# brownvc/matryodshka

Measured on AMD Instinct MI355X. Metric: novel-view frames/sec, 640x320 ODS->32-sphere MSI infer+render, higher is better.
Workload: dtype f32

## Files before the change

include/msi_hip.h:

```cpp
#ifndef MSI_HIP_H
#define MSI_HIP_H

#include <stddef.h>
#include <stdint.h>

#ifdef __cplusplus
extern "C" {
#endif

#define MSI_OK 0
#define MSI_E_BADARG (-1)
#define MSI_E_LAUNCH (-2)
#define MSI_E_UNSUPPORTED (-3)
#define MSI_E_WORKSPACE (-4)
#define MSI_E_RANGE (-5)

typedef void *msi_stream_t;

const char *msi_version(void);
#define MSI_ABI_VERSION 9
int32_t msi_abi_version(void);
const char *msi_last_error_string(void);
uint32_t msi_crc32c_host(const void *data_host, size_t n, uint32_t crc);

// ... 150 lines not shown
  uint64_t param_offset;
  uint64_t param_floats;
  uint64_t raw_offset;
  uint64_t affine_offset;
  uint64_t ln_scale_offset;
} msi_layer_info;

int msi_net_layer_info(const msi_net_desc *desc, int32_t layer, msi_layer_info *out);
size_t msi_net_param_floats(const msi_net_desc *desc);
size_t msi_net_packed_floats(const msi_net_desc *desc);
int msi_net_pack_weights_host(const msi_net_desc *desc, const float *params_host,
                              float *packed_host);
size_t msi_net_workspace_bytes(const msi_net_desc *desc);

typedef struct msi_net_plan msi_net_plan;
#define MSI_NET_OPT_FIXUP_KERNEL 0
#define MSI_NET_OPT_TAILSPLIT 1
#define MSI_NET_OPT_BIGTILE 2
#define MSI_NET_OPT_HEAD_FUSE_LN 3
#define MSI_NET_OPT_NUM_CUS 4
#define MSI_NET_OPT_F32_TILE 5
#define MSI_NET_OPT_F32_TILE_MASK 6
#define MSI_NET_OPT_APPLY_AHEAD 7
#define MSI_NET_OPT_HALO 8
#define MSI_NET_OPT_HALO_SKIP 9
#define MSI_NET_OPT_UNIFORM_SPLIT 10
#define MSI_NET_OPT_BF16_STAGE_RAW 11
#define MSI_NET_OPT_SPLIT_OVERHEAD 12
#define MSI_NET_OPT_BF16_WAVES 13
#define MSI_NET_OPT_F32_SPLIT3 14
#define MSI_NET_OPT_F32_SPLIT_F16 15
#define MSI_NET_OPT_X3_TILE8 16
#define MSI_NET_OPT_X3_ROWPAR 17
#define MSI_NET_OPT_COUNT 18
int msi_net_plan_create(const msi_net_desc *desc, msi_net_plan **out_plan);
void msi_net_plan_destroy(msi_net_plan *plan);
int msi_net_plan_set_option(msi_net_plan *plan, int32_t option, int32_t value);
size_t msi_net_plan_workspace_bytes(const msi_net_plan *plan);
int32_t msi_net_plan_layer_is_normalized(const msi_net_plan *plan, int32_t layer);
int32_t msi_net_plan_layer_kernel(const msi_net_plan *plan, int32_t layer, char *name, size_t name_bytes, int32_t *nblocks,
                                  int32_t *nsplit_tiles);
int32_t msi_net_plan_layer_params(const msi_net_plan *plan, int32_t layer, void *out, size_t bytes, size_t *needed);
#define MSI_NET_STATUS_APPLY_AHEAD_TIMEOUT 1
#define MSI_NET_STATUS_LN_OVERFLOW 2
#define MSI_NET_STATUS_LN_UNDERFLOW 4
#define MSI_NET_STATUS_F16_SPLIT_RANGE 8
int32_t msi_net_plan_status(const msi_net_plan *plan, const void *workspace, msi_stream_t stream, int32_t *status_bits);
int32_t msi_net_plan_calibrate(const msi_net_plan *plan, float *packed, const void *net_input, void *workspace, size_t workspace_bytes,
                               msi_stream_t stream, int32_t *layers_changed);
int msi_net_plan_forward(const msi_net_plan *plan, const float *packed, const void *net_input, float *pred,
                         void *workspace, size_t workspace_bytes, msi_stream_t stream);

int msi_net_plan_forward_rgba(const msi_net_plan *plan, const float *packed, const void *net_input, float *rgba_native,
                              float *blend_weights, float *alphas, float *pred, void *workspace, size_t workspace_bytes,
                              msi_stream_t stream, void *event_after_convs);

int msi_net_plan_forward_layers(const msi_net_plan *plan, const float *packed, const void *net_input, float *rgba_native,
                                void *layers_out, int32_t format, float *blend_weights, float *alphas, float *pred,
                                void *workspace, size_t workspace_bytes, msi_stream_t stream, void *event_after_convs);

int msi_net_forward_f32(const msi_net_desc *desc, const float *packed, const float *net_input,
                        float *pred, void *workspace, size_t workspace_bytes,
                        msi_stream_t stream);
int msi_net_forward_bf16(const msi_net_desc *desc, const float *packed, const void *net_input_bf16,
                         float *pred, void *workspace, size_t workspace_bytes,
                         msi_stream_t stream);

// ... 5 lines not shown
```

matryodshka_amd/_native.py:

```python
import ctypes
import os
from ctypes import POINTER, Structure, c_char, c_char_p, c_float, c_int32, c_size_t, c_uint64, c_void_p

_HERE = os.path.dirname(os.path.abspath(__file__))
LIB_PATH = os.path.join(_HERE, "libmsi_hip.so")

MSI_OK = 0
MSI_NET_NUM_LAYERS = 18
RENDER_STATUS_ORIGIN_OUTSIDE = 1
MSI_CAMERA_EQUIRECT, MSI_CAMERA_PINHOLE = 0, 1
MSI_LAYERS_F32, MSI_LAYERS_RGBA8, MSI_LAYERS_RGBA16F = 0, 1, 2
MSI_SCORE_F32, MSI_SCORE_U8 = 0, 1
MSI_SCORE_RAW, MSI_SCORE_IMAGE, MSI_SCORE_DEPTH = 0, 1, 2
MSI_SCORE_MSE, MSI_SCORE_MAE, MSI_SCORE_SSIM = 1, 2, 4
MSI_ABI_VERSION = 9


class MsiError(RuntimeError):
    pass


class NetDesc(Structure):
    _fields_ = [("batch", c_int32), ("height", c_int32), ("width", c_int32),
                ("in_channels", c_int32), ("num_outputs", c_int32), ("ngf", c_int32),
                ("coord_net", c_int32), ("dtype", c_int32)]


MSI_DTYPE_F32, MSI_DTYPE_BF16 = 0, 1
NET_OPT_FIXUP_KERNEL, NET_OPT_TAILSPLIT, NET_OPT_BIGTILE, NET_OPT_HEAD_FUSE_LN, NET_OPT_NUM_CUS = 0, 1, 2, 3, 4
NET_OPT_F32_TILE, NET_OPT_F32_TILE_MASK, NET_OPT_APPLY_AHEAD, NET_OPT_HALO, NET_OPT_HALO_SKIP = 5, 6, 7, 8, 9
NET_OPT_UNIFORM_SPLIT, NET_OPT_BF16_STAGE_RAW, NET_OPT_SPLIT_OVERHEAD, NET_OPT_BF16_WAVES, NET_OPT_F32_SPLIT3 = 10, 11, 12, 13, 14
NET_OPT_F32_SPLIT_F16 = 15
NET_OPT_X3_TILE8 = 16
NET_OPT_X3_ROWPAR = 17
NET_STATUS_F16_SPLIT_RANGE = 8


class LayerInfo(Structure):
    _fields_ = [("name", c_char * 16), ("kind", c_int32), ("cin", c_int32), ("cout", c_int32),
                ("has_coord", c_int32), ("stride", c_int32), ("rate", c_int32),
                ("in_h", c_int32), ("in_w", c_int32), ("out_h", c_int32), ("out_w", c_int32),
                ("param_offset", c_uint64), ("param_floats", c_uint64),
                ("raw_offset", c_uint64), ("affine_offset", c_uint64), ("ln_scale_offset", c_uint64)]


_P = c_void_p
_I = c_int32

SIGNATURES = {
    "msi_version": (c_char_p, []),
    "msi_abi_version": (c_int32, []),
    "msi_last_error_string": (c_char_p, []),
    "msi_crc32c_host": (ctypes.c_uint32, [_P, c_size_t, ctypes.c_uint32]),
    "msi_probe_matrix_rate": (_I, [_I, ctypes.c_int64, _I, _P, _P, _P]),
    "msi_trig_table_floats": (c_size_t, [_I, _I]),
    "msi_build_trig_tables_host": (_I, [_I, _I, _P]),
    "msi_preprocess_u8_f32": (_I, [_P, _P, c_size_t, _P]),
    "msi_preprocess_pair_u8_f32": (_I, [_P, _P, _P, _P, c_size_t, _P]),
    "msi_deprocess_pair_f32_u8": (_I, [_P, _P, _P, _P, c_size_t, _P]),
    "msi_preprocess_f32": (_I, [_P, _P, c_size_t, _P]),
    "msi_deprocess_f32_u8": (_I, [_P, _P, c_size_t, _I, _P]),
    "msi_compose_poses_f32": (_I, [_P, _P, _P, _I, _P]),
    "msi_ods_sphere_sweep_f32": (_I, [_P, _P, _P, _P, _P, _I, _I, _I, _I, _I, _P, _I, _I, _P]),
    "msi_ods_sphere_sweep_bf16": (_I, [_P, _P, _P, _P, _P, _I, _I, _I, _I, _I, _P, _I, _I, _P]),
    "msi_ods_sweep_volume": (_I, [_P, _P, _P, _P, _P, _P, _P, _I, _I, _I, _I, _P, _I, _P]),
    "msi_compose_pose_pair_f32": (_I, [_P, _P, _P, _P, _P, _I, _P]),
    "msi_assemble_rgba_f32": (_I, [_P, _P, _P, _P, _P, _I, _I, _I, _I, _P]),
# ... 111 lines not shown
```

matryodshka_amd/csrc/cnn.hip:

```cpp
#include "cnn_plan.h"

namespace msi_cnn {

int device_cu_count() {
  int dev = 0;
  hipDeviceProp_t prop;
  if (hipGetDevice(&dev) != hipSuccess || hipGetDeviceProperties(&prop, dev) != hipSuccess || prop.multiProcessorCount <= 0) {
    (void)hipGetLastError();
    return DEFAULT_CUS;
  }
  return prop.multiProcessorCount;
}

int launch_conv(const LayerLaunch &Q, const ConvParams &p, hipStream_t stream) {
  const ConvVariant &V = Q.variant;
  int rc;
  switch (V.family) {
    case CONV_IGEMM: rc = launch_igemm(Q, p, stream); break;
    case CONV_HALO: case CONV_HALO_S2: case CONVT_HALO: rc = launch_halo_f32(Q, p, stream); break;
    case CONV_HALO_X3: case CONV_HALO8_X3: case CONV_HALO_S2_X3: case CONV_HALO8_S2_X3: case CONVT_HALO_X3: case CONVT_HALO8_X3: rc = launch_x3(Q, p, stream); break;
    case CONV_HALO_BF16: case CONV_HALO_BF16_S2: case CONVT_HALO_BF16: rc = launch_bf16_halo(Q, p, stream); break;
    default: return msi::fail(MSI_E_UNSUPPORTED, "conv: unknown kernel family %d", V.family);
  }
  if (rc || Q.nfix == 0 || p.tile_cnt != nullptr) return rc;
// ... 216 lines not shown
static int forward_fused_tail(const char *who, const msi_net_plan *plan, const float *packed, const void *net_input, float *rgba_native,
                              void *layers_out, int32_t format, float *blend_weights, float *alphas, float *pred, void *workspace,
                              size_t workspace_bytes, msi_stream_t stream_, void *event_after_convs) {
  MSI_REQUIRE(plan, "%s: null plan", who);
  const msi_net_desc *desc = &plan->desc;
  const Net &net = plan->net;
  const Layer &H = net.layers[MSI_NET_NUM_LAYERS - 1];
  const int nd = desc->num_outputs / 2;
  const int bf16 = desc->dtype == MSI_DTYPE_BF16;
  if ((!bf16 && !plan->launch[MSI_NET_NUM_LAYERS - 1].fuse_ln) || (bf16 && !plan->opt[MSI_NET_OPT_HEAD_FUSE_LN]) ||
      H.c0 > 64 || H.c0 % 4 != 0 || desc->num_outputs != 2 * nd || nd % 4 != 0 || nd > 64 || desc->in_channels != 6 * nd ||
      ((long)desc->height * desc->width) % HA_TP != 0)
    return msi::fail(MSI_E_UNSUPPORTED, "%s: fused tail needs a blend_psv network (in = 6 D, out = 2 D, "
                     "D %% 4 == 0, D <= 64, ngf <= 64, HEAD_FUSE_LN on)", who);
  MSI_REQUIRE(rgba_native || layers_out, "%s: null pointer", who);
  MSI_REQUIRE(!layers_out || (reinterpret_cast<uintptr_t>(layers_out) & 15) == 0, "%s: layers_out is not 16-byte aligned", who);
  const int ng = (nd + HA_LG - 1) / HA_LG;
  if (nd % ng != 0 || (nd / ng) % 4 != 0 || (ng > 1 && bf16 && (nd / ng) % 8 != 0))
    return msi::fail(MSI_E_UNSUPPORTED, "%s: D = %d does not split into layer groups of a multiple of %d", who, nd, bf16 ? 8 : 4);
  int rc = run_layers(plan, packed, net_input, nullptr, workspace, workspace_bytes, stream_, MSI_NET_NUM_LAYERS - 1);
  if (rc || desc->batch == 0) return rc;
  hipStream_t stream = msi::as_stream(stream_);
  if (event_after_convs) {
    hipError_t e = hipEventRecord(static_cast<hipEvent_t>(event_after_convs), stream);
    if (e != hipSuccess) return msi::fail(MSI_E_LAUNCH, "%s: %s", who, hipGetErrorString(e));
  }
  char *ws = static_cast<char *>(workspace);
  const Layer &S = net.layers[H.src0];
  HeadAsmParams q;
  q.x = reinterpret_cast<const float *>(ws + S.raw_off);
  q.wpk = packed + H.packed_off;
  q.bias = packed + H.gamma_off;
  float *aff = reinterpret_cast<float *>(ws + S.aff_off);
  rc = launch_ln_finish(desc->batch, stream, reinterpret_cast<const long long *>(ws + S.sums_off), 1.0 / S.ln_count,
                        reinterpret_cast<const double *>(packed + S.lnscl_off), reinterpret_cast<int *>(ws + net.err_off),
                        packed + S.gamma_off, packed + S.beta_off, S.cout, aff, bf16);
  if (rc) return rc;
  q.aff = aff;
  q.psv = net_input;
  q.rgba = reinterpret_cast<float4 *>(rgba_native);
  q.layers = layers_out;
  q.bw_out = blend_weights;
  q.al_out = alphas;
  q.pred_out = pred;
  q.C0 = H.c0; q.ksteps = H.ksteps; q.npad = H.npad;
  q.nd = nd; q.hw = desc->height * desc->width;
  q.npix_total = (long)desc->batch * q.hw;
  q.lg = nd / ng;
  q.ng = ng;
  {
    auto magic = [](unsigned d) { return d == 1 ? 0xffffffffu : (unsigned)((1ull << 32) / d); };
    const int vec = bf16 ? 8 : 4;
    const unsigned vpp = (unsigned)((ng == 1 ? 6 * nd : 2 * 3 * q.lg) / vec);
    q.mg_vpp = magic(vpp);
    q.mg_nchunk = magic((unsigned)(q.ksteps * 8));
    q.mg_hw = magic((unsigned)q.hw);
    if (q.npix_total >= (1L << 32)) return msi::fail(MSI_E_UNSUPPORTED, "%s: more than 2^32 pixels per batch", who);
  }
  constexpr int BN = 64;
  size_t r_bytes = (size_t)q.ksteps * (HA_TP + BN) * ROW_BYTES;
  if (r_bytes < (size_t)HA_TP * (6 * q.lg + 1) * sizeof(float)) r_bytes = (size_t)HA_TP * (6 * q.lg + 1) * sizeof(float);
  if (bf16) {
    r_bytes = (size_t)q.ksteps * HA_TP * ROW_BYTES;
    if (r_bytes < (size_t)HA_TP * (3 * q.lg + 1) * sizeof(unsigned)) r_bytes = (size_t)HA_TP * (3 * q.lg + 1) * sizeof(unsigned);
  }
  const size_t lds = 2 * 64 * 4 + 64 + ((r_bytes + 15) & ~(size_t)15) + (size_t)HA_TP * (2 * q.lg + 1) * sizeof(float);
  const long ntile = q.npix_total / HA_TP;
  if (((ntile + 7) / 8) * 8 * ng >= (1L << 31)) return msi::fail(MSI_E_UNSUPPORTED, "%s: too many pixel tiles for one launch", who);
  return launch_head_assemble(bf16, layers_out ? format : MSI_LAYERS_F32, (unsigned)(((ntile + 7) / 8) * 8 * ng), lds, stream, q);
}

int msi_net_plan_forward_rgba(const msi_net_plan *plan, const float *packed, const void *net_input, float *rgba_native,
                              float *blend_weights, float *alphas, float *pred, void *workspace, size_t workspace_bytes,
                              msi_stream_t stream_, void *event_after_convs) {
  return forward_fused_tail("net_forward_rgba", plan, packed, net_input, rgba_native, nullptr, MSI_LAYERS_F32, blend_weights, alphas, pred,
                            workspace, workspace_bytes, stream_, event_after_convs);
}

int msi_net_plan_forward_layers(const msi_net_plan *plan, const float *packed, const void *net_input, float *rgba_native,
                                void *layers_out, int32_t format, float *blend_weights, float *alphas, float *pred, void *workspace,
                                size_t workspace_bytes, msi_stream_t stream_, void *event_after_convs) {
  MSI_REQUIRE(!layers_out || format == MSI_LAYERS_RGBA8 || format == MSI_LAYERS_RGBA16F,
              "net_forward_layers: unknown format %d (layers_out is MSI_LAYERS_RGBA8 or MSI_LAYERS_RGBA16F)", format);
  MSI_REQUIRE(rgba_native || layers_out, "net_forward_layers: null pointer");
  return forward_fused_tail("net_forward_layers", plan, packed, net_input, rgba_native, layers_out, format, blend_weights, alphas, pred,
                            workspace, workspace_bytes, stream_, event_after_convs);
}

size_t msi_net_workspace_bytes(const msi_net_desc *desc) {
  msi_net_plan *pl = nullptr;
  if (msi_net_plan_create(desc, &pl)) return 0;
  const size_t n = pl->net.ws_bytes;
  msi_net_plan_destroy(pl);
  return n;
}

static int forward_once(const msi_net_desc *desc, const float *packed, const void *net_input, float *pred,
                        void *workspace, size_t workspace_bytes, msi_stream_t stream) {
  msi_net_plan *pl = nullptr;
  int rc = msi_net_plan_create(desc, &pl);
  if (rc) return rc;
// ... 19 lines not shown
```

matryodshka_amd/csrc/cnn_device.h:

```cpp
#pragma once
#include <cmath>
#include <cstdint>
#include <cstdio>
#include <cstdlib>
#include <cstring>
#include <new>
#include <type_traits>
#include <vector>

#include "msi_common.h"

namespace msi_cnn {


typedef float f32x16 __attribute__((ext_vector_type(16)));
typedef float v4f __attribute__((ext_vector_type(4)));
typedef __attribute__((address_space(3))) void lds_void;

constexpr int BK = 32;
constexpr int ROW_BYTES = BK * 4;
#ifndef MSI_NSTAGE
#define MSI_NSTAGE 2
#endif
constexpr int NSTAGE = MSI_NSTAGE;
// ... 86 lines not shown

struct LayerLaunch {
  ConvParams p;
  ConvVariant variant;
  int nblocks, nfix;
  int inlaunch;
  int fuse_ln;
  int skip_apply;
  unsigned ln_blocks;
};

constexpr int HA_TP = 32;
#ifndef MSI_HA_LG
#define MSI_HA_LG 32
#endif
constexpr int HA_LG = MSI_HA_LG;

struct HeadAsmParams {
  const float *x;
  const float *wpk;
  const float *bias;
  const float *aff;
  const void *psv;
  float4 *rgba;
  float *bw_out, *al_out;
  float *pred_out;
  int C0, ksteps, npad, nd, hw;
  int lg, ng;
  unsigned mg_vpp, mg_nchunk, mg_hw;
  long npix_total;
  void *layers;
};

int launch_conv(const LayerLaunch &Q, const ConvParams &p, hipStream_t stream);
int launch_igemm(const LayerLaunch &Q, const ConvParams &p, hipStream_t stream);
int launch_fixup(int bm, int bn, int mode, int raw16, unsigned grid_x, unsigned grid_y, const ConvParams &p, hipStream_t stream);
int launch_halo_f32(const LayerLaunch &Q, const ConvParams &p, hipStream_t stream);
int launch_x3(const LayerLaunch &Q, const ConvParams &p, hipStream_t stream);
int launch_bf16_halo(const LayerLaunch &Q, const ConvParams &p, hipStream_t stream);
int launch_zero(void *p, size_t n16, hipStream_t stream);
int launch_ln_finish(int batch, hipStream_t stream, const long long *sums, double inv_n, const double *scl, int *status, const float *gamma, const float *beta, int C,
                     float *aff, int raw16);
int launch_ln_apply(int bf16out, unsigned blocks, int batch, size_t lds, hipStream_t stream, float *x, const long long *sums, double inv_n, const double *scl, int *status,
                    const float *gamma, const float *beta, size_t per_sample, int C, float *aff, unsigned short *yb);
int launch_head_assemble(int bf16in, int format, unsigned grid_x, size_t lds, hipStream_t stream, const HeadAsmParams &q);
int debug_conv_occupancy(int lds_bytes);

constexpr int vkey(int family, int a = 0, int b = 0, int c = 0, int d = 0, int e = 0) { return ((((family * 16 + a) * 16 + b) * 16 + c) * 16 + d) * 16 + e; }

inline int set_max_lds(const void *fn, int lds, unsigned long long &done, const char *what) {
  int dev = 0;
  if (hipGetDevice(&dev) != hipSuccess) dev = 0;
  const bool tracked = dev >= 0 && dev < 64;
  if (tracked && ((done >> dev) & 1ull)) return MSI_OK;
  hipError_t e = hipFuncSetAttribute(fn, hipFuncAttributeMaxDynamicSharedMemorySize, lds);
  if (e != hipSuccess) return msi::fail(MSI_E_LAUNCH, "%s: %s", what, hipGetErrorString(e));
  if (tracked) done |= 1ull << dev;
  return MSI_OK;
}

template <auto KERNEL, int LDS, int THREADS = 256>
int launch_kernel(unsigned nblocks, const ConvParams &p, hipStream_t stream, const char *what) {
  if constexpr (LDS > 65536) {
    static thread_local unsigned long long done = 0;
    int rc0 = set_max_lds(reinterpret_cast<const void *>(KERNEL), LDS, done, what);
    if (rc0) return rc0;
  }
  hipLaunchKernelGGL(KERNEL, dim3(nblocks), dim3(THREADS), LDS, stream, p);
  return msi::check_launch(what);
}

template <int N> using IC = std::integral_constant<int, N>;
}
using namespace msi_cnn;

namespace {

template <int MODE>
// ... 636 lines not shown
```

matryodshka_amd/csrc/cnn_plan.hip:

```cpp
#include "cnn_plan.h"

namespace {

void plan_tiles(ConvParams &p, int BM, int BN, int batch, int num_cus, int tailsplit, int max_split, int *nblocks, int *nfix,
                int uniform_split = 0, int split_overhead = 0, bool split_any_tile = false) {
  const int mtot = p.Mh * p.Mw;
  p.tiles_m = (mtot + BM - 1) / BM;
  if (p.halo_tx) p.tiles_m = ((p.Mh + BM / 16 - 1) / (BM / 16)) * p.halo_tx;
  p.tiles_n = (p.Cout + BN - 1) / BN;
  p.ntiles = p.tiles_m * p.tiles_n * p.nclass * batch;
  p.n_main = p.ntiles;
  p.split0 = 1;
  p.split = 1;
  const int Q = CONV_SLOTS_PER_CU * num_cus;
  if (BM * BN == 64 * 64 && tailsplit == 2 && p.ntiles >= Q && p.ntiles % Q != 0 && p.ksteps >= 2 * MAX_SPLIT) {
    const int remq = p.ntiles % Q;
    int best = 1;
    double best_cost = 1.0;
    for (int sp = 2; sp <= max_split; ++sp) {
      if ((long)remq * sp > 2L * num_cus * MAX_SPLIT) break;
      const double cost = (double)((remq * sp + Q - 1) / Q) / sp;
      if (cost < best_cost - 1e-9) { best_cost = cost; best = sp; }
    }
    if (best > 1) { p.split = best; p.n_main = p.ntiles - remq; }
// ... 226 lines not shown
    }
  }
  return MSI_OK;
}

}

extern "C" {

int msi_net_plan_create(const msi_net_desc *desc, msi_net_plan **out) {
  MSI_REQUIRE(desc && out, "net_plan_create: null pointer");
  *out = nullptr;
  msi_net_plan *pl = new (std::nothrow) msi_net_plan();
  if (!pl) return msi::fail(MSI_E_WORKSPACE, "net_plan_create: out of host memory");
  pl->desc = *desc;
  pl->num_cus = device_cu_count();
  pl->opt[MSI_NET_OPT_FIXUP_KERNEL] = 0;
  pl->opt[MSI_NET_OPT_TAILSPLIT] = 1;
  pl->opt[MSI_NET_OPT_BIGTILE] = 1;
  pl->opt[MSI_NET_OPT_HEAD_FUSE_LN] = 1;
  pl->opt[MSI_NET_OPT_NUM_CUS] = pl->num_cus;
  pl->opt[MSI_NET_OPT_APPLY_AHEAD] = 0;
  pl->opt[MSI_NET_OPT_HALO] = 5;
  pl->opt[MSI_NET_OPT_F32_TILE] = 0;
  pl->opt[MSI_NET_OPT_F32_TILE_MASK] = 0;
  pl->opt[MSI_NET_OPT_UNIFORM_SPLIT] = 0;
  pl->opt[MSI_NET_OPT_SPLIT_OVERHEAD] = 0;
  pl->opt[MSI_NET_OPT_BF16_WAVES] = 8;
  pl->opt[MSI_NET_OPT_F32_SPLIT_F16] = 0;
  pl->opt[MSI_NET_OPT_X3_TILE8] = 0x3ffff;
  pl->opt[MSI_NET_OPT_X3_ROWPAR] = 0x3ffff;
  pl->opt[MSI_NET_OPT_F32_SPLIT3] = 0x3ffff;
  pl->opt[MSI_NET_OPT_BF16_STAGE_RAW] = 1;
  int rc = plan_layers(pl);
  if (rc) { delete pl; return rc; }
  *out = pl;
  return MSI_OK;
}

void msi_net_plan_destroy(msi_net_plan *plan) { delete plan; }

int msi_net_plan_set_option(msi_net_plan *plan, int32_t option, int32_t value) {
  MSI_REQUIRE(plan, "net_plan_set_option: null plan");
  MSI_REQUIRE(option >= 0 && option < MSI_NET_OPT_COUNT, "net_plan_set_option: unknown option %d", option);
  if (option == MSI_NET_OPT_NUM_CUS) {
    MSI_REQUIRE(value >= 8 && value <= 4096, "net_plan_set_option: num_cus %d out of range", value);
    plan->num_cus = value;
  }
  if (option == MSI_NET_OPT_BIGTILE) MSI_REQUIRE(value >= 0 && value <= 2, "net_plan_set_option: bigtile %d", value);
  if (option == MSI_NET_OPT_HALO) MSI_REQUIRE(value >= 0 && value <= 7, "net_plan_set_option: halo %d (bit 0 conv, bit 1 conv-transpose, bit 2 stride-2 conv)", value);
  if (option == MSI_NET_OPT_TAILSPLIT) MSI_REQUIRE(value >= 0 && value <= 2, "net_plan_set_option: tailsplit %d", value);
  if (option == MSI_NET_OPT_F32_TILE) MSI_REQUIRE(value >= 0 && value <= 2, "net_plan_set_option: f32 tile %d", value);
  if (option == MSI_NET_OPT_BF16_WAVES) MSI_REQUIRE(value == 4 || value == 8, "net_plan_set_option: bf16 waves %d (4 or 8)", value);
#ifndef MSI_EXPERIMENTS
  if ((option == MSI_NET_OPT_F32_TILE || option == MSI_NET_OPT_F32_TILE_MASK || option == MSI_NET_OPT_APPLY_AHEAD) && value != 0)
    return msi::fail(MSI_E_UNSUPPORTED, "net_plan_set_option: option %d is an experiment this library was not built with "
                     "(MSI_CNN_DEFINES=-DMSI_EXPERIMENTS python -m matryodshka_amd.build --force)", option);
#endif
  const int old = plan->opt[option];
  plan->opt[option] = value;
  int rc = plan_layers(plan);
  if (rc) {
    plan->opt[option] = old;
    if (option == MSI_NET_OPT_NUM_CUS) plan->num_cus = old;
    plan_layers(plan);
  }
  return rc;
}

size_t msi_net_plan_workspace_bytes(const msi_net_plan *plan) { return plan ? plan->net.ws_bytes : 0; }

int32_t msi_net_plan_layer_is_normalized(const msi_net_plan *plan, int32_t layer) {
  if (!plan || layer < 0 || layer >= MSI_NET_NUM_LAYERS - 1) return -1;
  return plan->launch[layer].skip_apply ? 0 : 1;
}

int32_t msi_net_plan_layer_kernel(const msi_net_plan *plan, int32_t layer, char *name, size_t name_bytes, int32_t *nblocks,
                                  int32_t *nsplit_tiles) {
  MSI_REQUIRE(plan && name && name_bytes > 0, "net_plan_layer_kernel: null pointer");
  MSI_REQUIRE(layer >= 0 && layer < MSI_NET_NUM_LAYERS, "net_plan_layer_kernel: bad layer %d", layer);
  const LayerLaunch &Q = plan->launch[layer];
  const ConvVariant &V = Q.variant;
  switch (V.family) {
    case CONV_IGEMM: snprintf(name, name_bytes, "conv_igemm_kernel<%d, %d, %d, %d>", V.bm, V.bn, V.mode, V.bf16); break;
    case CONV_HALO: snprintf(name, name_bytes, "conv_halo_kernel<%d, %d>", V.rate, V.apply); break;
// ... 33 lines not shown
```

matryodshka_amd/csrc/cnn_tail.hip:

```cpp
#include "cnn_device.h"

namespace {


template <int BF16IN>
__global__ void __launch_bounds__(256) __attribute__((amdgpu_waves_per_eu(BF16IN ? 6 : 5)))
head_assemble_kernel(const HeadAsmParams p) {
  [[maybe_unused]] constexpr int FMT = MSI_LAYERS_F32;
#include "cnn_tail_head_assemble.inc"
}

template <int BF16IN, int FMT>
__global__ void __launch_bounds__(256) __attribute__((amdgpu_waves_per_eu(BF16IN ? 6 : 5)))
head_assemble_packed_kernel(const HeadAsmParams p) {
  static_assert(FMT == MSI_LAYERS_RGBA8 || FMT == MSI_LAYERS_RGBA16F, "a packed texel format");
#include "cnn_tail_head_assemble.inc"
}

__global__ void __launch_bounds__(256)
ln_finish_kernel(const long long *__restrict__ sums, double inv_n, const double *__restrict__ scl, int *status,
                 const float *__restrict__ gamma, const float *__restrict__ beta, int C, float *__restrict__ aff, int raw16) {
  __shared__ double s_stat[2];
  const int b = blockIdx.x, tid = threadIdx.x;
  ln_mean_inv(sums + (size_t)b * LN_SHARDS * LN_WORDS, inv_n, scl, status, s_stat, tid);
  const double mu = s_stat[0], inv = s_stat[1];
  const double up = raw16 ? scl[2] * 16777216.0 : 1.0;
  for (int c = tid; c < C; c += 256) {
    const double sc = inv * (double)gamma[c];
    aff[(size_t)b * 2 * C + c] = (float)(sc * up);
    aff[(size_t)b * 2 * C + C + c] = (float)((double)beta[c] - mu * sc);
  }
}

__global__ void __launch_bounds__(256) zero_kernel(float4 *__restrict__ p, size_t n16) {
  const size_t i = (size_t)blockIdx.x * 256 + threadIdx.x;
  if (i < n16) p[i] = float4{0.f, 0.f, 0.f, 0.f};
}

template <int BF16OUT>
__global__ void __launch_bounds__(256)
ln_apply_kernel(float *__restrict__ x, const long long *__restrict__ sums, double inv_n, const double *__restrict__ scl,
                int *status, const float *__restrict__ gamma, const float *__restrict__ beta, size_t per_sample, int C,
                float *__restrict__ aff, unsigned short *__restrict__ yb) {
  extern __shared__ __attribute__((aligned(16))) float s_aff[];
  __shared__ double s_stat[2];
  const int b = blockIdx.y, tid = threadIdx.x;
  ln_mean_inv(sums + (size_t)b * LN_SHARDS * LN_WORDS, inv_n, scl, (blockIdx.x == 0 ? status : nullptr), s_stat, tid);
  const double mu = s_stat[0], inv = s_stat[1];
  const double up = BF16OUT ? scl[2] * 16777216.0 : 1.0;
// ... 55 lines not shown
  hipLaunchKernelGGL(zero_kernel, dim3((unsigned)((n16 + 255) / 256)), dim3(256), 0, stream, reinterpret_cast<float4 *>(ptr), n16);
  return msi::check_launch("zero");
}
int launch_ln_finish(int batch, hipStream_t stream, const long long *sums, double inv_n, const double *scl, int *status, const float *gamma, const float *beta, int C,
                     float *aff, int raw16) {
  hipLaunchKernelGGL(ln_finish_kernel, dim3(batch), dim3(256), 0, stream, sums, inv_n, scl, status, gamma, beta, C, aff, raw16);
  return msi::check_launch("ln_finish");
}
int launch_ln_apply(int bf16out, unsigned blocks, int batch, size_t lds, hipStream_t stream, float *x, const long long *sums, double inv_n, const double *scl, int *status,
                    const float *gamma, const float *beta, size_t per_sample, int C, float *aff, unsigned short *yb) {
  const dim3 grid(blocks, batch);
  if (bf16out) hipLaunchKernelGGL(ln_apply_kernel<1>, grid, dim3(256), lds, stream, x, sums, inv_n, scl, status, gamma, beta, per_sample, C, aff, yb);
  else hipLaunchKernelGGL(ln_apply_kernel<0>, grid, dim3(256), lds, stream, x, sums, inv_n, scl, status, gamma, beta, per_sample, C, aff, yb);
  return msi::check_launch("ln_apply");
}
int launch_head_assemble(int bf16in, int format, unsigned grid_x, size_t lds, hipStream_t stream, const HeadAsmParams &q) {
#define MSI_LAUNCH_HA(K) hipLaunchKernelGGL(K, dim3(grid_x), dim3(256), lds, stream, q)
  switch (format) {
    case MSI_LAYERS_F32:
      if (bf16in) MSI_LAUNCH_HA(head_assemble_kernel<1>); else MSI_LAUNCH_HA(head_assemble_kernel<0>);
      break;
    case MSI_LAYERS_RGBA8:
      if (bf16in) MSI_LAUNCH_HA((head_assemble_packed_kernel<1, MSI_LAYERS_RGBA8>)); else MSI_LAUNCH_HA((head_assemble_packed_kernel<0, MSI_LAYERS_RGBA8>));
      break;
    case MSI_LAYERS_RGBA16F:
      if (bf16in) MSI_LAUNCH_HA((head_assemble_packed_kernel<1, MSI_LAYERS_RGBA16F>)); else MSI_LAUNCH_HA((head_assemble_packed_kernel<0, MSI_LAYERS_RGBA16F>));
      break;
    default:
      return msi::fail(MSI_E_BADARG, "head_assemble: unknown format %d", format);
  }
#undef MSI_LAUNCH_HA
  return msi::check_launch("head_assemble");
}
}
```

Before: 551.4.

## Add persistent head-assemble kernel that fuses LN finish and prefetches next tile

```diff
diff --git a/include/msi_hip.h b/include/msi_hip.h
--- a/include/msi_hip.h
+++ b/include/msi_hip.h
@@ -206,7 +206,8 @@
 #define MSI_NET_OPT_F32_SPLIT_F16 15
 #define MSI_NET_OPT_X3_TILE8 16
 #define MSI_NET_OPT_X3_ROWPAR 17
-#define MSI_NET_OPT_COUNT 18
+#define MSI_NET_OPT_TAIL_PERSIST 18
+#define MSI_NET_OPT_COUNT 19
 int msi_net_plan_create(const msi_net_desc *desc, msi_net_plan **out_plan);
 void msi_net_plan_destroy(msi_net_plan *plan);
 int msi_net_plan_set_option(msi_net_plan *plan, int32_t option, int32_t value);
diff --git a/matryodshka_amd/_native.py b/matryodshka_amd/_native.py
--- a/matryodshka_amd/_native.py
+++ b/matryodshka_amd/_native.py
@@ -33,6 +33,7 @@
 NET_OPT_F32_SPLIT_F16 = 15
 NET_OPT_X3_TILE8 = 16
 NET_OPT_X3_ROWPAR = 17
+NET_OPT_TAIL_PERSIST = 18
 NET_STATUS_F16_SPLIT_RANGE = 8
 
 
diff --git a/matryodshka_amd/csrc/cnn.hip b/matryodshka_amd/csrc/cnn.hip
--- a/matryodshka_amd/csrc/cnn.hip
+++ b/matryodshka_amd/csrc/cnn.hip
@@ -272,10 +272,17 @@
   q.wpk = packed + H.packed_off;
   q.bias = packed + H.gamma_off;
   float *aff = reinterpret_cast<float *>(ws + S.aff_off);
-  rc = launch_ln_finish(desc->batch, stream, reinterpret_cast<const long long *>(ws + S.sums_off), 1.0 / S.ln_count,
-                        reinterpret_cast<const double *>(packed + S.lnscl_off), reinterpret_cast<int *>(ws + net.err_off),
-                        packed + S.gamma_off, packed + S.beta_off, S.cout, aff, bf16);
-  if (rc) return rc;
+  const long ha_ntile = (long)desc->batch * desc->height * desc->width / HA_TP;
+  const long ha_full = ((ha_ntile + 7) / 8) * 8 * ng, ha_round = 8L * ng;
+  long ha_grid = (((long)(bf16 ? HAP_WPC_BF16 : HAP_WPC_F32) * plan->num_cus + ha_round - 1) / ha_round) * ha_round;
+  if (ha_grid > ha_full) ha_grid = ha_full;
+  const bool persist = plan->opt[MSI_NET_OPT_TAIL_PERSIST] != 0 && !(bf16 && ha_full > HAP_BF16_MAX_ROUNDS * ha_grid);
+  if (!persist) {
+    rc = launch_ln_finish(desc->batch, stream, reinterpret_cast<const long long *>(ws + S.sums_off), 1.0 / S.ln_count,
+                          reinterpret_cast<const double *>(packed + S.lnscl_off), reinterpret_cast<int *>(ws + net.err_off),
+                          packed + S.gamma_off, packed + S.beta_off, S.cout, aff, bf16);
+    if (rc) return rc;
+  }
   q.aff = aff;
   q.psv = net_input;
   q.rgba = reinterpret_cast<float4 *>(rgba_native);
@@ -307,6 +314,25 @@
   const size_t lds = 2 * 64 * 4 + 64 + ((r_bytes + 15) & ~(size_t)15) + (size_t)HA_TP * (2 * q.lg + 1) * sizeof(float);
   const long ntile = q.npix_total / HA_TP;
   if (((ntile + 7) / 8) * 8 * ng >= (1L << 31)) return msi::fail(MSI_E_UNSUPPORTED, "%s: too many pixel tiles for one launch", who);
+  if (persist) {
+    HeadAsmPersistParams pq;
+    pq.h = q;
+    const long grid = ha_grid;
+    pq.ntile = ntile;
+    pq.tile_step = grid / ng;
+    pq.ln_sums = reinterpret_cast<const long long *>(ws + S.sums_off);
+    pq.ln_scl = reinterpret_cast<const double *>(packed + S.lnscl_off);
+    pq.ln_inv_n = 1.0 / S.ln_count;
+    pq.ln_gamma = packed + S.gamma_off;
+    pq.ln_beta = packed + S.beta_off;
+    pq.aff_out = aff;
+    pq.status = reinterpret_cast<int *>(ws + net.err_off);
+    size_t pr_bytes = (size_t)q.ksteps * HA_TP * ROW_BYTES;
+    const size_t psv_bytes = bf16 ? (size_t)HA_TP * (3 * q.lg + 1) * sizeof(unsigned) : (size_t)HA_TP * (6 * q.lg + 1) * sizeof(float);
+    if (pr_bytes < psv_bytes) pr_bytes = psv_bytes;
+    const size_t plds = 2 * 64 * 4 + 64 + 64 * 4 + ((pr_bytes + 15) & ~(size_t)15) + (size_t)HA_TP * (2 * q.lg + 1) * sizeof(float);
+    return launch_head_assemble_persist(bf16, layers_out ? format : MSI_LAYERS_F32, (unsigned)grid, plds, stream, pq);
+  }
   return launch_head_assemble(bf16, layers_out ? format : MSI_LAYERS_F32, (unsigned)(((ntile + 7) / 8) * 8 * ng), lds, stream, q);
 }
 
diff --git a/matryodshka_amd/csrc/cnn_device.h b/matryodshka_amd/csrc/cnn_device.h
--- a/matryodshka_amd/csrc/cnn_device.h
+++ b/matryodshka_amd/csrc/cnn_device.h
@@ -142,6 +142,23 @@
   void *layers;
 };
 
+#ifndef MSI_HAP_BF16_WPC
+#define MSI_HAP_BF16_WPC 5
+#endif
+constexpr long HAP_BF16_MAX_ROUNDS = 16;
+constexpr int HAP_WPC_F32 = 4, HAP_WPC_BF16 = MSI_HAP_BF16_WPC;
+struct HeadAsmPersistParams {
+  HeadAsmParams h;
+  long ntile;
+  long tile_step;
+  const long long *ln_sums;
+  const double *ln_scl;
+  double ln_inv_n;
+  const float *ln_gamma, *ln_beta;
+  float *aff_out;
+  int *status;
+};
+
 int launch_conv(const LayerLaunch &Q, const ConvParams &p, hipStream_t stream);
 int launch_igemm(const LayerLaunch &Q, const ConvParams &p, hipStream_t stream);
 int launch_fixup(int bm, int bn, int mode, int raw16, unsigned grid_x, unsigned grid_y, const ConvParams &p, hipStream_t stream);
@@ -154,6 +171,7 @@
 int launch_ln_apply(int bf16out, unsigned blocks, int batch, size_t lds, hipStream_t stream, float *x, const long long *sums, double inv_n, const double *scl, int *status,
                     const float *gamma, const float *beta, size_t per_sample, int C, float *aff, unsigned short *yb);
 int launch_head_assemble(int bf16in, int format, unsigned grid_x, size_t lds, hipStream_t stream, const HeadAsmParams &q);
+int launch_head_assemble_persist(int bf16in, int format, unsigned grid_x, size_t lds, hipStream_t stream, const HeadAsmPersistParams &q);
 int debug_conv_occupancy(int lds_bytes);
 
 constexpr int vkey(int family, int a = 0, int b = 0, int c = 0, int d = 0, int e = 0) { return ((((family * 16 + a) * 16 + b) * 16 + c) * 16 + d) * 16 + e; }
diff --git a/matryodshka_amd/csrc/cnn_plan.hip b/matryodshka_amd/csrc/cnn_plan.hip
--- a/matryodshka_amd/csrc/cnn_plan.hip
+++ b/matryodshka_amd/csrc/cnn_plan.hip
@@ -282,6 +282,7 @@
   pl->opt[MSI_NET_OPT_X3_ROWPAR] = 0x3ffff;
   pl->opt[MSI_NET_OPT_F32_SPLIT3] = 0x3ffff;
   pl->opt[MSI_NET_OPT_BF16_STAGE_RAW] = 1;
+  pl->opt[MSI_NET_OPT_TAIL_PERSIST] = 1;
   int rc = plan_layers(pl);
   if (rc) { delete pl; return rc; }
   *out = pl;
@@ -301,6 +302,7 @@
   if (option == MSI_NET_OPT_HALO) MSI_REQUIRE(value >= 0 && value <= 7, "net_plan_set_option: halo %d (bit 0 conv, bit 1 conv-transpose, bit 2 stride-2 conv)", value);
   if (option == MSI_NET_OPT_TAILSPLIT) MSI_REQUIRE(value >= 0 && value <= 2, "net_plan_set_option: tailsplit %d", value);
   if (option == MSI_NET_OPT_F32_TILE) MSI_REQUIRE(value >= 0 && value <= 2, "net_plan_set_option: f32 tile %d", value);
+  if (option == MSI_NET_OPT_TAIL_PERSIST) MSI_REQUIRE(value == 0 || value == 1, "net_plan_set_option: tail persist %d (0 or 1)", value);
   if (option == MSI_NET_OPT_BF16_WAVES) MSI_REQUIRE(value == 4 || value == 8, "net_plan_set_option: bf16 waves %d (4 or 8)", value);
 #ifndef MSI_EXPERIMENTS
   if ((option == MSI_NET_OPT_F32_TILE || option == MSI_NET_OPT_F32_TILE_MASK || option == MSI_NET_OPT_APPLY_AHEAD) && value != 0)
diff --git a/matryodshka_amd/csrc/cnn_tail.hip b/matryodshka_amd/csrc/cnn_tail.hip
--- a/matryodshka_amd/csrc/cnn_tail.hip
+++ b/matryodshka_amd/csrc/cnn_tail.hip
@@ -15,6 +15,20 @@
 head_assemble_packed_kernel(const HeadAsmParams p) {
   static_assert(FMT == MSI_LAYERS_RGBA8 || FMT == MSI_LAYERS_RGBA16F, "a packed texel format");
 #include "cnn_tail_head_assemble.inc"
+}
+
+template <int BF16IN>
+__global__ void __launch_bounds__(256) __attribute__((amdgpu_waves_per_eu(BF16IN ? HAP_WPC_BF16 : HAP_WPC_F32)))
+head_assemble_persist_kernel(const HeadAsmPersistParams pp) {
+  [[maybe_unused]] constexpr int FMT = MSI_LAYERS_F32;
+#include "cnn_tail_head_assemble_persist.inc"
+}
+
+template <int BF16IN, int FMT>
+__global__ void __launch_bounds__(256) __attribute__((amdgpu_waves_per_eu(BF16IN ? HAP_WPC_BF16 : HAP_WPC_F32)))
+head_assemble_persist_packed_kernel(const HeadAsmPersistParams pp) {
+  static_assert(FMT == MSI_LAYERS_RGBA8 || FMT == MSI_LAYERS_RGBA16F, "a packed texel format");
+#include "cnn_tail_head_assemble_persist.inc"
 }
 
 __global__ void __launch_bounds__(256)
@@ -136,4 +150,22 @@
 #undef MSI_LAUNCH_HA
   return msi::check_launch("head_assemble");
 }
+int launch_head_assemble_persist(int bf16in, int format, unsigned grid_x, size_t lds, hipStream_t stream, const HeadAsmPersistParams &q) {
+#define MSI_LAUNCH_HAP(K) hipLaunchKernelGGL(K, dim3(grid_x), dim3(256), lds, stream, q)
+  switch (format) {
+    case MSI_LAYERS_F32:
+      if (bf16in) MSI_LAUNCH_HAP(head_assemble_persist_kernel<1>); else MSI_LAUNCH_HAP(head_assemble_persist_kernel<0>);
+      break;
+    case MSI_LAYERS_RGBA8:
+      if (bf16in) MSI_LAUNCH_HAP((head_assemble_persist_packed_kernel<1, MSI_LAYERS_RGBA8>)); else MSI_LAUNCH_HAP((head_assemble_persist_packed_kernel<0, MSI_LAYERS_RGBA8>));
+      break;
+    case MSI_LAYERS_RGBA16F:
+      if (bf16in) MSI_LAUNCH_HAP((head_assemble_persist_packed_kernel<1, MSI_LAYERS_RGBA16F>)); else MSI_LAUNCH_HAP((head_assemble_persist_packed_kernel<0, MSI_LAYERS_RGBA16F>));
+      break;
+    default:
+      return msi::fail(MSI_E_BADARG, "head_assemble_persist: unknown format %d", format);
+  }
+#undef MSI_LAUNCH_HAP
+  return msi::check_launch("head_assemble_persist");
 }
+}
diff --git a/matryodshka_amd/csrc/cnn_tail_head_assemble_persist.inc b/matryodshka_amd/csrc/cnn_tail_head_assemble_persist.inc
--- /dev/null
+++ b/matryodshka_amd/csrc/cnn_tail_head_assemble_persist.inc
@@ -0,0 +1,282 @@
+#if defined(__HIP_DEVICE_COMPILE__)
+  const HeadAsmParams &p = pp.h;
+  extern __shared__ __attribute__((aligned(16))) char smem[];
+  const int tid = threadIdx.x, lane = tid & 63, wave = tid >> 6;
+  const int nd = p.nd, lg = p.lg, ng = p.ng;
+  const unsigned slot = blockIdx.x >> 3;
+  const unsigned tsl = ng == 1 ? slot : (ng == 2 ? slot >> 1 : slot / (unsigned)ng);
+  const int g = (int)(slot - tsl * (unsigned)ng);
+  long tile = (long)tsl * 8 + (blockIdx.x & 7u);
+  if (tile >= pp.ntile) return;
+  const int c_psv = 6 * nd, c_pred = 2 * nd;
+  const int l_cpsv = 6 * lg, l_cpred = 2 * lg;
+  const int s_psv = l_cpsv + 1, s_pred = l_cpred + 1;
+  const int s_psv16 = 3 * lg + 1;
+  float *s_aff = reinterpret_cast<float *>(smem);
+  double *s_stat = reinterpret_cast<double *>(smem + 2 * 64 * 4);
+  float *s_bias = reinterpret_cast<float *>(smem + 2 * 64 * 4 + 64);
+  char *sR = smem + 2 * 64 * 4 + 64 + 64 * 4;
+  char *sA = sR;
+  const size_t r_bytes = BF16IN ? max((size_t)p.ksteps * HA_TP * ROW_BYTES, (size_t)HA_TP * s_psv16 * sizeof(unsigned))
+                                : max((size_t)p.ksteps * HA_TP * ROW_BYTES, (size_t)HA_TP * s_psv * sizeof(float));
+  float *l_psv = reinterpret_cast<float *>(sR);
+  float *l_pred = reinterpret_cast<float *>(sR + ((r_bytes + 15) & ~(size_t)15));
+  auto gcol = [&](int n) __attribute__((always_inline)) -> int { return n < lg ? g * lg + n : nd + g * lg + (n - lg); };
+
+  constexpr int PSV_PER_THREAD = BF16IN ? 3 : 6;
+  constexpr int PSV_VEC = BF16IN ? 8 : 4;
+  constexpr int ESZ = BF16IN ? 2 : 4;
+  const int nrun = ng == 1 ? 1 : 2;
+  const int run_len = ng == 1 ? c_psv : 3 * lg;
+  const int vpr = run_len / PSV_VEC, vpp = nrun * vpr;
+  const int nv_psv = HA_TP * vpp;
+  const int nchunk = p.ksteps * 8;
+
+  constexpr int NWF = BF16IN ? 4 : 8;
+  v4f wfrag[NWF];
+  if (wave < 2) {
+    const int frow = lane & 31, fh = lane >> 5;
+    const int nloc = wave * 32 + frow;
+    const int gn = gcol(nloc < l_cpred ? nloc : 0);
+    const int fswz = (gn >> 1) & 7;
+#pragma unroll
+    for (int i = 0; i < NWF; ++i) {
+      wfrag[i] = v4f{0.f, 0.f, 0.f, 0.f};
+      if (BF16IN) {
+        if (nloc < l_cpred)
+          wfrag[i] = *reinterpret_cast<const v4f *>(p.wpk + (size_t)gn * (ROW_BYTES / 4) + (((2 * i + fh) ^ fswz) << 2));
+      } else {
+        const int ks = i >> 2, qq = i & 3;
+        if (ks < p.ksteps && nloc < l_cpred)
+          wfrag[i] = *reinterpret_cast<const v4f *>(p.wpk + ((size_t)ks * p.npad + gn) * (ROW_BYTES / 4) + (((fh * 4 + qq) ^ fswz) << 2));
+      }
+    }
+  }
+  if (tid < 64) s_bias[tid] = tid < l_cpred ? p.bias[gcol(tid)] : 0.f;
+  float ln_ga = 0.f, ln_be = 0.f;
+  if (tid < p.C0) { ln_ga = pp.ln_gamma[tid]; ln_be = pp.ln_beta[tid]; }
+
+  float4 q[PSV_PER_THREAD];
+  v4f araw[2];
+  auto request = [&](long pt, int tid) __attribute__((always_inline)) {
+    if (BF16IN) {
+      const int r = tid >> 3, c = (tid & 7) * 8;
+      araw[0] = v4f{0.f, 0.f, 0.f, 0.f};
+      if (c < p.C0) araw[0] = *reinterpret_cast<const v4f *>(reinterpret_cast<const _Float16 *>(p.x) + (size_t)(pt + r) * p.C0 + c);
+    } else {
+#pragma unroll
+      for (int k = 0; k < 2; ++k) {
+        const int e = tid + 256 * k;
+        const int r = (int)udiv_magic((unsigned)e, (unsigned)nchunk, p.mg_nchunk), c = (e - r * nchunk) * 4;
+        araw[k] = v4f{0.f, 0.f, 0.f, 0.f};
+        if (e < HA_TP * nchunk && c < p.C0) araw[k] = *reinterpret_cast<const v4f *>(p.x + (size_t)(pt + r) * p.C0 + c);
+      }
+    }
+    const char *gp = static_cast<const char *>(p.psv) + (size_t)pt * c_psv * ESZ;
+#pragma unroll
+    for (int k = 0; k < PSV_PER_THREAD; ++k) {
+      const int v = tid + 256 * k;
+      if (v < nv_psv) {
+        if (ng == 1) {
+          q[k] = reinterpret_cast<const float4 *>(gp)[v];
+        } else {
+          const int px = (int)udiv_magic((unsigned)v, (unsigned)vpp, p.mg_vpp), w = v - px * vpp;
+          const int r = w >= vpr ? 1 : 0, idx = w - r * vpr;
+          const int start = r == 0 ? 3 * g * lg : 3 * (nd + g * lg);
+          q[k] = *reinterpret_cast<const float4 *>(gp + ((size_t)px * c_psv + start + idx * PSV_VEC) * ESZ);
+        }
+      }
+    }
+  };
+
+  long p0 = tile * HA_TP;
+  int b = (int)udiv_magic((unsigned)p0, (unsigned)p.hw, p.mg_hw);
+  LnShard shard = ln_shard_load(pp.ln_sums + (size_t)b * LN_SHARDS * LN_WORDS, tid);
+  request(p0, tid);
+  bool need_ln = true;
+
+  for (;;) {
+    int tid_tile = tid;
+    asm volatile("" : "+v"(tid_tile));
+    {
+    const int tid = tid_tile, lane = tid_tile & 63, wave = tid_tile >> 6;
+    if (need_ln) {
+      const bool owner = g == 0 && p0 == (long)b * p.hw;
+      ln_mean_inv_pre(shard, pp.ln_inv_n, pp.ln_scl, owner ? pp.status : nullptr, s_stat, tid);
+      const double mu = s_stat[0], inv = s_stat[1];
+      const double up = BF16IN ? pp.ln_scl[2] * 16777216.0 : 1.0;
+      if (tid < p.C0) {
+        const double sc = inv * (double)ln_ga;
+        const float fs = (float)(sc * up), ft = (float)((double)ln_be - mu * sc);
+        s_aff[tid] = fs;
+        s_aff[p.C0 + tid] = ft;
+        if (owner) {
+          pp.aff_out[(size_t)b * 2 * p.C0 + tid] = fs;
+          pp.aff_out[(size_t)b * 2 * p.C0 + p.C0 + tid] = ft;
+        }
+      }
+    }
+    __syncthreads();
+    if (BF16IN) {
+      typedef _Float16 h8_t __attribute__((ext_vector_type(8)));
+      const int r = tid >> 3, ch = tid & 7, c = ch * 8;
+      unsigned pk[4] = {0u, 0u, 0u, 0u};
+      if (c < p.C0) {
+        const h8_t h = __builtin_bit_cast(h8_t, araw[0]);
+        const v4f a2[2] = {v4f{(float)h[0], (float)h[1], (float)h[2], (float)h[3]}, v4f{(float)h[4], (float)h[5], (float)h[6], (float)h[7]}};
+        float y[8];
+#pragma unroll
+        for (int k = 0; k < 2; ++k) {
+          const v4f s4 = *reinterpret_cast<const v4f *>(s_aff + c + 4 * k), t4 = *reinterpret_cast<const v4f *>(s_aff + p.C0 + c + 4 * k);
+          y[4 * k] = fmaxf(a2[k].x * s4.x + t4.x, 0.f); y[4 * k + 1] = fmaxf(a2[k].y * s4.y + t4.y, 0.f);
+          y[4 * k + 2] = fmaxf(a2[k].z * s4.z + t4.z, 0.f); y[4 * k + 3] = fmaxf(a2[k].w * s4.w + t4.w, 0.f);
+        }
+#pragma unroll
+        for (int k = 0; k < 4; ++k) asm("v_cvt_pk_bf16_f32 %0, %1, %2" : "=v"(pk[k]) : "v"(y[2 * k]), "v"(y[2 * k + 1]));
+      }
+      typedef unsigned v4u_t __attribute__((ext_vector_type(4)));
+      *reinterpret_cast<v4u_t *>(sA + r * ROW_BYTES + ((ch ^ ((r >> 1) & 7)) << 4)) = v4u_t{pk[0], pk[1], pk[2], pk[3]};
+    } else
+#pragma unroll
+    for (int k = 0; k < 2; ++k) {
+      const int e = tid + 256 * k;
+      if (e < HA_TP * nchunk) {
+        const int r = (int)udiv_magic((unsigned)e, (unsigned)nchunk, p.mg_nchunk), ch = e - r * nchunk;
+        const int c = ch * 4;
+        v4f y = {0.f, 0.f, 0.f, 0.f};
+        if (c < p.C0) {
+          const v4f s4 = *reinterpret_cast<const v4f *>(s_aff + c), t4 = *reinterpret_cast<const v4f *>(s_aff + p.C0 + c);
+          y.x = fmaxf(araw[k].x * s4.x + t4.x, 0.f); y.y = fmaxf(araw[k].y * s4.y + t4.y, 0.f);
+          y.z = fmaxf(araw[k].z * s4.z + t4.z, 0.f); y.w = fmaxf(araw[k].w * s4.w + t4.w, 0.f);
+        }
+        const int ks = ch >> 3, chunk = ch & 7;
+        *reinterpret_cast<v4f *>(sA + (ks * HA_TP + r) * ROW_BYTES + ((chunk ^ ((r >> 1) & 7)) << 4)) = y;
+      }
+    }
+    __syncthreads();
+    if (wave < 2) {
+      f32x16 acc;
+#pragma unroll
+      for (int r = 0; r < 16; ++r) acc[r] = 0.f;
+      const int frow = lane & 31, fh = lane >> 5;
+      const int fswz_a = (frow >> 1) & 7;
+      if (BF16IN) {
+        typedef __bf16 bf16x8 __attribute__((ext_vector_type(8)));
+#pragma unroll
+        for (int qq = 0; qq < 4; ++qq) {
+          const v4f a = *reinterpret_cast<const v4f *>(sA + frow * ROW_BYTES + (((2 * qq + fh) ^ fswz_a) << 4));
+          acc = __builtin_amdgcn_mfma_f32_32x32x16_bf16(__builtin_bit_cast(bf16x8, wfrag[qq]), __builtin_bit_cast(bf16x8, a), acc, 0, 0, 0);
+        }
+      } else {
+#pragma unroll
+        for (int ks = 0; ks < 2; ++ks) {
+          if (ks < p.ksteps) {
+#pragma unroll
+            for (int qq = 0; qq < 4; ++qq) {
+              const v4f a = *reinterpret_cast<const v4f *>(sA + (ks * HA_TP + frow) * ROW_BYTES + (((fh * 4 + qq) ^ fswz_a) << 4));
+              const v4f w = wfrag[(ks * 4 + qq) % NWF];
+              acc = __builtin_amdgcn_mfma_f32_32x32x2f32(w.x, a.x, acc, 0, 0, 0);
+              acc = __builtin_amdgcn_mfma_f32_32x32x2f32(w.y, a.y, acc, 0, 0, 0);
+              acc = __builtin_amdgcn_mfma_f32_32x32x2f32(w.z, a.z, acc, 0, 0, 0);
+              acc = __builtin_amdgcn_mfma_f32_32x32x2f32(w.w, a.w, acc, 0, 0, 0);
+            }
+          }
+        }
+      }
+      const int px = lane & 31, half = lane >> 5;
+#pragma unroll
+      for (int gg = 0; gg < 4; ++gg) {
+        const int n = wave * 32 + 8 * gg + 4 * half;
+        if (n < l_cpred) {
+          const int gn = gcol(n);
+          const v4f bs = *reinterpret_cast<const v4f *>(s_bias + n);
+          v4f t = {msi_tanh(acc[4 * gg] + bs.x), msi_tanh(acc[4 * gg + 1] + bs.y), msi_tanh(acc[4 * gg + 2] + bs.z), msi_tanh(acc[4 * gg + 3] + bs.w)};
+          if (p.pred_out) *reinterpret_cast<v4f *>(p.pred_out + (p0 + px) * c_pred + gn) = t;
+          t.x = (t.x + 1.0f) / 2.0f; t.y = (t.y + 1.0f) / 2.0f; t.z = (t.z + 1.0f) / 2.0f; t.w = (t.w + 1.0f) / 2.0f;
+          float *dst = l_pred + px * s_pred + n;
+          dst[0] = t.x; dst[1] = t.y; dst[2] = t.z; dst[3] = t.w;
+          if (n < lg) {
+            if (p.bw_out) *reinterpret_cast<v4f *>(p.bw_out + (p0 + px) * nd + gn) = t;
+          } else {
+            if (p.al_out) *reinterpret_cast<v4f *>(p.al_out + (p0 + px) * nd + (gn - nd)) = t;
+          }
+        }
+      }
+    }
+    __syncthreads();
+#pragma unroll
+    for (int k = 0; k < PSV_PER_THREAD; ++k) {
+      const int v = tid + 256 * k;
+      if (v < nv_psv) {
+        const int px = (int)udiv_magic((unsigned)v, (unsigned)vpp, p.mg_vpp), w = v - px * vpp;
+        if (BF16IN) {
+          unsigned *dst = reinterpret_cast<unsigned *>(l_psv) + px * s_psv16 + w * 4;
+          dst[0] = __builtin_bit_cast(unsigned, q[k].x); dst[1] = __builtin_bit_cast(unsigned, q[k].y);
+          dst[2] = __builtin_bit_cast(unsigned, q[k].z); dst[3] = __builtin_bit_cast(unsigned, q[k].w);
+        } else {
+          float *dst = l_psv + px * s_psv + w * PSV_VEC;
+          dst[0] = q[k].x; dst[1] = q[k].y; dst[2] = q[k].z; dst[3] = q[k].w;
+        }
+      }
+    }
+    const long tile_n = tile + pp.tile_step;
+    const bool more = tile_n < pp.ntile;
+    const long p0_n = tile_n * HA_TP;
+    int b_n = b;
+    need_ln = false;
+    if (more) {
+      b_n = (int)udiv_magic((unsigned)p0_n, (unsigned)p.hw, p.mg_hw);
+      if (b_n != b) {
+        shard = ln_shard_load(pp.ln_sums + (size_t)b_n * LN_SHARDS * LN_WORDS, tid);
+        need_ln = true;
+      }
+      request(p0_n, tid);
+    }
+    __syncthreads();
+    {
+#pragma clang fp contract(off)
+      const int px = tid & (HA_TP - 1);
+      const long pq = p0 + px;
+      const long off = pq - (long)b * p.hw;
+      const float *rp = l_psv + px * s_psv;
+      const float *rq = l_pred + px * s_pred;
+      float4 *dst = p.rgba + ((long)b * nd + g * lg + tid / HA_TP) * p.hw + off;
+      const long dstep = (long)(256 / HA_TP) * p.hw;
+      constexpr int TEXEL_BYTES = FMT == MSI_LAYERS_RGBA8 ? 4 : 8;
+      char *dstp = FMT != MSI_LAYERS_F32 ? static_cast<char *>(p.layers) + (((long)b * nd + g * lg + tid / HA_TP) * p.hw + off) * TEXEL_BYTES : nullptr;
+      const bool want_f32 = FMT == MSI_LAYERS_F32 || p.rgba != nullptr;
+      const unsigned *rp16 = reinterpret_cast<const unsigned *>(l_psv) + px * s_psv16;
+      for (int d = tid / HA_TP; d < lg; d += 256 / HA_TP, dst += dstep, dstp += dstep * TEXEL_BYTES) {
+        float fgv[3], bgv[3];
+        if (BF16IN) {
+          const int ef = 3 * d, eb = 3 * (lg + d);
+          const unsigned f0 = rp16[ef >> 1], f1 = rp16[(ef >> 1) + 1], b0 = rp16[eb >> 1], b1 = rp16[(eb >> 1) + 1];
+          const unsigned long long fw = ((unsigned long long)f1 << 32 | f0) >> ((ef & 1) * 16), bw = ((unsigned long long)b1 << 32 | b0) >> ((eb & 1) * 16);
+#pragma unroll
+          for (int c = 0; c < 3; ++c) {
+            fgv[c] = __builtin_bit_cast(float, (unsigned)(fw >> (16 * c)) << 16);
+            bgv[c] = __builtin_bit_cast(float, (unsigned)(bw >> (16 * c)) << 16);
+          }
+        } else {
+#pragma unroll
+          for (int c = 0; c < 3; ++c) { fgv[c] = rp[d * 3 + c]; bgv[c] = rp[(lg + d) * 3 + c]; }
+        }
+        const float *fg = fgv;
+        const float *bg = bgv;
+        const float w = rq[d];
+        const float omw = 1.0f - w;
+        float4 o;
+        o.x = w * fg[0] + omw * bg[0];
+        o.y = w * fg[1] + omw * bg[1];
+        o.z = w * fg[2] + omw * bg[2];
+        o.w = rq[lg + d];
+        if constexpr (FMT == MSI_LAYERS_RGBA8) *reinterpret_cast<unsigned *>(dstp) = rgba8_encode(o);
+        else if constexpr (FMT == MSI_LAYERS_RGBA16F) *reinterpret_cast<u32x2_g *>(dstp) = rgba16f_encode(o);
+        if (want_f32) *dst = o;
+      }
+    }
+    if (!more) break;
+    tile = tile_n; p0 = p0_n; b = b_n;
+    }
+  }
+#endif
```

Result: no change. 555.2, median of 6 (+0.7%).
